# B10532021/Part-Aware_Measurement_for_3D_Pose_Estimation_and_Tracking

Hardware: AMD Instinct MI355X
Metric: multi-view frames/sec (end-to-end: HRNet-W48 2D pose + part-aware cross-view matching + DLT tracking) (higher is better)
Workload: dtype bf16 convs / f64 matching

## Files before the change

include/pam.h:

```cpp
#ifndef PAM_H
#define PAM_H

#include <stddef.h>
#include <stdint.h>

#ifdef __cplusplus
extern "C" {
#endif

#define PAM_J 17
#define PAM_MAX_VIEWS 32
#define PAM_MAX_TAPS 16
#define PAM_EXP_TABLE 64
#define PAM_YOLO_MAX_CAND 1024

#define PAM_OK 0
#define PAM_E_ARG (-1)
#define PAM_E_HIP (-2)
#define PAM_E_STATE (-3)
#define PAM_E_OVERFLOW (-4)

typedef struct PamParams {
    double conf_threshold;
    double epi_threshold;
// ... 105 lines not shown
                            const int32_t* dev_view_of, const float* dev_boxes, int out_h, int out_w, int out_c, void* dev_out_bf16,
                            int antialias);
int pam_preprocess_crops_flip(void* stream, int n, int n_total, const void* const* dev_frames, int frame_h, int frame_w,
                              const int32_t* dev_view_of, const float* dev_boxes, int out_h, int out_w, int out_c, void* dev_out_bf16,
                              int antialias);
int pam_preprocess_crops_affine(void* stream, int n, int n_total, int flip, const void* const* dev_frames, int frame_h, int frame_w,
                                const int32_t* dev_view_of, const float* dev_boxes, float box_scale, int out_h, int out_w, int out_c,
                                void* dev_out_bf16, int antialias, float* dev_eff_xywh);
int pam_box_cs(void* stream, int n, const float* dev_boxes, int out_w, int out_h, float box_scale, float* dev_eff_xywh);
int pam_box_cs_host(int n, const float* boxes, int out_w, int out_h, float box_scale, float* eff);
#define PAM_FLIP_MERGE 1
#define PAM_FLIP_SHIFT 2
#define PAM_FLIP_QUARTER 4
long long pam_head_decode_flip_scratch_bytes(int n, int hm_h, int hm_w);
int pam_head_decode_flip(void* stream, int n, int flip_row0, int hm_h, int hm_w, const void* feat_bf16, int C, const float* w,
                         const float* bias, int J, int flags, float* dev_heatmaps_or_null, const int32_t* dev_view_of,
                         const int32_t* dev_slot_of, const float* dev_boxes, int max_dets, double* dev_det, float* dev_kp_xyc,
                         void* dev_scratch);
long long pam_head_decode_dark_scratch_bytes(int n, int hm_h, int hm_w);
int pam_head_decode_dark(void* stream, int n, int flip_row0, int hm_h, int hm_w, const void* feat_bf16, int C, const float* w,
                         const float* bias, int J, int flags, int blur_kernel, float* dev_heatmaps_or_null, const int32_t* dev_view_of,
                         const int32_t* dev_slot_of, const float* dev_boxes, int max_dets, double* dev_det, float* dev_kp_xyc,
                         void* dev_scratch);
int pam_decode_heatmaps(void* stream, int n, const float* dev_heatmaps, int nchw, int hm_h, int hm_w,
                        const int32_t* dev_view_of, const int32_t* dev_slot_of, const float* dev_boxes,
                        int max_dets, double* dev_det, float* dev_kp_xyc );
int pam_clock_probe(void* stream, unsigned long long* dev_out2, int microseconds);

int pam_conv2d_nhwc_bf16(void* stream, const void* in, const void* w_packed, const void* w_img, const float* bias,
                         const void* residual, void* out, int N, int H, int W, int Cin, int Cout, int KH, int KW,
                         int stride, int pad, int relu, int tile_cfg);
int pam_conv2d_nhwc_bf16_ex(void* stream, const void* in, const void* w_packed, const void* w_img, const float* bias,
                            const void* residual, void* out, int N, int H, int W, int Cin, int Cout, int KH, int KW,
                            int stride, int pad, int relu, int tile_cfg, int in_cstride, int relu_from);
int pam_conv3x3_slab(int H, int W, int Cin, int Cout);
int pam_conv3x3_layout(int H, int W, int Cin, int Cout);
int pam_conv3x3_layout_ex(int H, int W, int Cin, int Cout, int c96_slab);
int pam_conv3x3_layout_gen(int H, int W, int Cin, int Cout);
int pam_conv3x3_layout_small(int H, int W, int Cin, int Cout);
#define PAM_CONV_KERNEL_IGEMM 0
#define PAM_CONV_KERNEL_3X3   1
#define PAM_CONV_KERNEL_3X3S  2
#define PAM_CONV_KERNEL_GS    3
#define PAM_CONV_KERNEL_STEM  4
int pam_conv_last_kernel(void);
int pam_conv_last_form(void);
int pam_conv_plan(int N, int H, int W, int Cin, int Cout, int KH, int KW, int stride, int pad, int relu, int tile_cfg, int in_cstride,
                  int relu_from, int has_in, int has_w_packed, int has_w_img, int has_residual, int has_out, int32_t* kernel, int32_t* form);
int pam_conv_debug_stamps(void* dev_buf);
int pam_upsample_add_nhwc_bf16(void* stream, const void* base, int n_terms, const void* const* terms,
                               const int32_t* shifts, void* out, int N, int H, int W, int C, int relu);
int pam_upsample_add_nhwc_bf16_ex(void* stream, const void* base, int n_terms, const void* const* terms, const int32_t* shifts,
                                  const int32_t* term_cstrides, void* out, int N, int H, int W, int C, int relu);

int pam_basic_block2_tile(int C, int N, int H, int W, int32_t* out2);
int pam_basic_block2_nhwc_bf16(void* stream, const void* in, const void* wpack, void* out, int N, int H, int W, int C,
                               int tile_rows, int tile_cols);

int pam_stem_fused_nhwc_bf16(void* stream, const void* in, const void* w1frag, const float* bias1, const void* w2img, const float* bias2,
                             const void* wp_img, const float* biasp, void* out_x0, void* out_y1, int N, int H, int W);
int pam_bottleneck_fused_nhwc_bf16(void* stream, const void* y1, const void* x0, const void* residual, const void* w2img,
                                   const float* bias2, const void* w3_img, const float* bias3, const void* w1_img, const float* bias1,
                                   void* out_x, void* out_y1, int N, int H, int W);
int pam_resnet_stem_nhwc_bf16(void* stream, const void* in, const void* wfrag, const float* bias, void* out, int N, int H, int W);
int pam_deconv4x4s2_nhwc_bf16(void* stream, const void* in, const void* wimg, const float* bias, void* out, int N, int H, int W,
                              int Cin, int Cout, int relu);
int pam_pointwise64_relu_nhwc_bf16(void* stream, const void* in, const void* w_img, const float* bias, void* out, long long n_pixels);
int pam_pointwise64_act_nhwc_bf16(void* stream, const void* in, const void* w_img, const float* bias, void* out, long long n_pixels, int act);
int pam_bottleneck_tail_nhwc_bf16(void* stream, const void* y2, const void* x0, const void* residual, const void* w3_img,
                                  const float* bias3, const void* w1_img, const float* bias1, void* out_x, void* out_y1,
                                  long long n_pixels, int tile_cfg);

int pam_conv3x3s2_c48_tile(int N, int H, int W, int Cout, int32_t* out3);
int pam_conv3x3s2_slab(int H, int W, int Cin, int Cout);
int pam_conv3x3s2_nhwc_bf16(void* stream, const void* in, int in_cstride, const void* w_img, const float* bias, void* out, int N, int H,
                            int W, int Cin, int Cout, int relu, int relu_from);
int pam_conv3x3s2_c48_nhwc_bf16(void* stream, const void* in, int in_cstride, const void* wpack, const float* bias, const void* res,
                                int res_cstride, void* out, int out_cstride, int N, int H, int W, int Cout, int relu, int relu_from,
                                int tile_rows, int tile_cols, int slab_groups);
int pam_fuse_sum_nhwc_bf16(void* stream, const void* base, int n_plain, const void* const* plain, const int32_t* plain_cstrides, int n_up,
                           const void* const* up_src, const int32_t* up_shifts, const int32_t* up_channels, const void* const* up_wimg,
                           const float* const* up_bias, void* out, int N, int H, int W, int C, int relu, int tile_a, int tile_b,
                           int max_workgroups);

int pam_flag_signal(void* stream, int32_t* dev_counter);
int pam_flag_signal_mask(void* stream, int32_t* dev_counters, uint32_t mask);
int pam_flag_gate(void* stream, int32_t* dev_counter, int target, int32_t* dev_err, const uint32_t* dev_max_us, int arrive, int32_t* host_err,
                  int32_t* dev_void);

int pam_comm_unique_id(void* id128);
int pam_comm_init(void** comm, int world, int rank, const void* id128, int device);
int pam_comm_destroy(void* comm);
const char* pam_comm_last_error(void);
int pam_allgather_keypoints(PamHandle* h, void* comm, void* stream, const double* dev_send, int rows_per_rank, double* dev_recv);

int pam_resize_frames(void* stream, int n, const void* const* dev_frames, int frame_h, int frame_w,
                      int out_h, int out_w, void* dev_out_bf16);
int pam_upsample_concat_nhwc_bf16(void* stream, const void* a, const void* b, void* out, int N, int H, int W, int Ca, int Cb);
int pam_yolo_detect(void* stream, int n_img, const void* const* heads , const int32_t* grid_h,
                    const int32_t* grid_w, const int32_t* chan_stride, const float* anchors, int net_w, int net_h,
                    int num_classes, int class_id, float score_thresh, float nms_thresh, int frame_w, int frame_h,
                    int max_det, float* dev_out, int32_t* dev_count);
long long pam_yolo_detect_workspace_bytes(int n_img, const int32_t* grid_h, const int32_t* grid_w);
int pam_yolo_detect_ws(void* stream, int n_img, const void* const* heads, const int32_t* grid_h, const int32_t* grid_w,
                       const int32_t* chan_stride, const float* anchors, int net_w, int net_h, int num_classes, int class_id,
                       float score_thresh, float nms_thresh, int frame_w, int frame_h, int max_det, float* dev_out, int32_t* dev_count,
                       void* dev_workspace, long long workspace_bytes);

long long pam_yolo_detect_heads_workspace_bytes(int n_img, int n_heads, const int32_t* grid_h, const int32_t* grid_w);
int pam_yolo_detect_heads(void* stream, int n_img, int n_heads, const void* const* heads, const int32_t* grid_h, const int32_t* grid_w,
                          const int32_t* chan_stride, const float* anchors, int net_w, int net_h, int num_classes, int class_id,
                          float score_thresh, float nms_thresh, int frame_w, int frame_h, int max_det, float* dev_out, int32_t* dev_count);
int pam_yolo_detect_heads_ws(void* stream, int n_img, int n_heads, const void* const* heads, const int32_t* grid_h, const int32_t* grid_w,
                             const int32_t* chan_stride, const float* anchors, int net_w, int net_h, int num_classes, int class_id,
                             float score_thresh, float nms_thresh, int frame_w, int frame_h, int max_det, float* dev_out, int32_t* dev_count,
                             void* dev_workspace, long long workspace_bytes);
int pam_maxpool_nhwc_bf16(void* stream, const void* in, void* out, int N, int H, int W, int C, int size, int stride);
#define PAM_SPP_MAX_HW 32
int pam_spp_concat_nhwc_bf16(void* stream, const void* in, void* out, int N, int H, int W, int C, int s1, int s2, int s3);
int pam_spp_concat_slab_nhwc_bf16(void* stream, const void* in, void* out, int N, int H, int W, int C, int s1, int s2, int s3, int slab);

#define PAM_JPEG_U_NOT_JPEG 1
#define PAM_JPEG_U_PROGRESSIVE 2
#define PAM_JPEG_U_ARITHMETIC 3
#define PAM_JPEG_U_SOF 4
#define PAM_JPEG_U_PRECISION 5
#define PAM_JPEG_U_QUANT16 6
#define PAM_JPEG_U_COMPONENTS 7
#define PAM_JPEG_U_COLORSPACE 8
#define PAM_JPEG_U_SAMPLING 9
#define PAM_JPEG_U_SCAN 10
#define PAM_JPEG_U_DNL 11

typedef struct PamJpegInfo {
    int32_t width, height, n_comp;
    int32_t unsupported;
    int32_t h_samp[3], v_samp[3];
    int32_t mcu_w, mcu_h;
    int32_t blocks_w[3], blocks_h[3];
    int32_t restart_interval;
    int32_t reserved;
    int64_t coef_offset[3];
    int64_t coef_words;
    uint16_t quant[3][64];
} PamJpegInfo;

int pam_jpeg_probe(const uint8_t* data, size_t n, PamJpegInfo* info);
int pam_jpeg_entropy(const uint8_t* data, size_t n, const PamJpegInfo* info, int16_t* coef, size_t coef_words);

typedef struct PamJpegImage {
    const int16_t* dev_coef;
    const uint16_t* dev_quant;
    uint8_t* dev_planes;
    uint8_t* dev_out;
    int32_t width, height, n_comp, h_samp, v_samp, reserved;
} PamJpegImage;

int pam_jpeg_reconstruct(void* stream, int n_img, const PamJpegImage* images);


typedef struct PamJpegFwdImage {
    const uint8_t* dev_bgr;
    const uint16_t* dev_quant;
    int16_t* dev_coef;
    int32_t width, height, h_samp, v_samp;
} PamJpegFwdImage;
// ... 46 lines not shown
```

part-aware_measurement_for_3d_pose_estimation_and_tracking_amd/_lib.py:

```python
import ctypes as C
import math
import os

import numpy as np

_HERE = os.path.dirname(os.path.abspath(__file__))
LIB_PATH = os.environ.get('PAM_LIB') or os.path.join(_HERE, 'csrc', 'libpam_hip.so')

PAM_J = 17
PAM_MAX_TAPS = 16
PAM_EXP_TABLE = 64


class PamParams(C.Structure):
    _fields_ = [
        ('conf_threshold', C.c_double), ('epi_threshold', C.c_double), ('init_threshold', C.c_double),
        ('joint_threshold', C.c_double), ('alpha2d', C.c_double), ('lambda_a', C.c_double), ('lambda_t', C.c_double),
        ('n_init', C.c_int32), ('max_age', C.c_int32), ('count_gate', C.c_int32), ('n_taps_body', C.c_int32),
        ('n_taps_arm', C.c_int32), ('reserved', C.c_int32),
        ('taps_body', C.c_double * PAM_MAX_TAPS), ('taps_arm', C.c_double * PAM_MAX_TAPS),
        ('exp_lambda_a', C.c_double * PAM_EXP_TABLE), ('w_lambda_t', C.c_double * 4),
    ]


# ... 26 lines not shown


class PamJpegEncodeParams(C.Structure):
    _fields_ = [('width', C.c_int32), ('height', C.c_int32), ('h_samp', C.c_int32), ('v_samp', C.c_int32),
                ('quality', C.c_int32), ('reserved', C.c_int32), ('quant', (C.c_uint16 * 64) * 2)]


class PamOverlayPrim(C.Structure):
    _fields_ = [('ax', C.c_int32), ('ay', C.c_int32), ('bx', C.c_int32), ('by', C.c_int32), ('hw', C.c_int32), ('bgr', C.c_uint32),
                ('reserved', C.c_int32 * 2)]


class PamOverlayView(C.Structure):
    _fields_ = [('dev_bgr', C.c_void_p), ('width', C.c_int32), ('height', C.c_int32), ('prim_first', C.c_int32), ('prim_count', C.c_int32)]


class PamOverlayTrackView(C.Structure):
    _fields_ = [('camera', C.c_int32), ('extra', C.c_int32), ('width', C.c_int32), ('height', C.c_int32)]


_P = C.c_void_p
_I = C.c_int
_SIGS = {
    'pam_create': (_I, [C.POINTER(_P), _I, _I, _I, _I, _I, _I, C.POINTER(PamParams)]),
    'pam_destroy': (_I, [_P]),
    'pam_last_error': (C.c_char_p, [_P]),
    'pam_version': (C.c_char_p, []),
    'pam_set_cameras': (_I, [_P, _P, _P, _P, _P]),
    'pam_reset': (_I, [_P]),
    'pam_out_layout': (_I, [_P, C.POINTER(PamOutLayout)]),
    'pam_frame_plan': (_I, [_P, _P, _P, _P]),
    'pam_frame': (_I, [_P, _I, _P, _P, _P, _P]),
    'pam_frame_dev': (_I, [_P, _P, _I, _P, _P]),
    'pam_frame_dev_views': (_I, [_P, _P, _I, _P, _P]),
    'pam_fetch': (_I, [_P, _P, _P, _P]),
    'pam_sync': (_I, [_P, _P]),
    'pam_op_project': (_I, [_P, _I, _I, _P, _P]),
    'pam_op_track_affinity': (_I, [_P, _I, _I, _I, _P, _P, _P, _P]),
    'pam_op_lsap': (_I, [_P, _I, _I, _P, _P, _P, _P]),
    'pam_op_epi_dist': (_I, [_P, _I, _P, _P, _P]),
    'pam_op_epi_pair': (_I, [_P, _I, _P, _I, _P, _P]),
    'pam_op_epi_dist_init': (_I, [_P, _I, _P, _P, _P]),
    'pam_op_greedy': (_I, [_P, _I, _I, _P, _P, _P, _P, _P]),
    'pam_op_dlt': (_I, [_P, _I, _P, _P, _P, _P, _P, _P]),
    'pam_op_dlt_paths': (_I, [_P, _I, _P, _P, _P, _P, _P, _I, _I, _P, _P]),
    'pam_op_smooth': (_I, [_P, _I, _P, _P, _P]),
    'pam_op_velocity': (_I, [_P, _I, _P, _P]),
    'pam_op_hyp_cost': (_I, [_P, _I, _P, _P, _I, _P, _P, _P]),
    'pam_preprocess_crops': (_I, [_P, _I, _P, _I, _I, _P, _P, _I, _I, _I, _P]),
    'pam_preprocess_crops_ex': (_I, [_P, _I, _I, _P, _I, _I, _P, _P, _I, _I, _I, _P, _I]),
    'pam_preprocess_crops_flip': (_I, [_P, _I, _I, _P, _I, _I, _P, _P, _I, _I, _I, _P, _I]),
    'pam_preprocess_crops_affine': (_I, [_P, _I, _I, _I, _P, _I, _I, _P, _P, C.c_float, _I, _I, _I, _P, _I, _P]),
    'pam_box_cs': (_I, [_P, _I, _P, _I, _I, C.c_float, _P]),
    'pam_box_cs_host': (_I, [_I, _P, _I, _I, C.c_float, _P]),
    'pam_decode_heatmaps': (_I, [_P, _I, _P, _I, _I, _I, _P, _P, _P, _I, _P, _P]),
    'pam_clock_probe': (_I, [_P, _P, _I]),
    'pam_conv2d_nhwc_bf16': (_I, [_P, _P, _P, _P, _P, _P, _P] + [_I] * 11),
    'pam_conv2d_nhwc_bf16_ex': (_I, [_P, _P, _P, _P, _P, _P, _P] + [_I] * 13),
    'pam_conv3x3_slab': (_I, [_I, _I, _I, _I]),
    'pam_conv3x3_layout': (_I, [_I, _I, _I, _I]),
    'pam_conv_last_kernel': (_I, []),
    'pam_conv_last_form': (_I, []),
    'pam_conv_plan': (_I, [_I] * 18 + [_P, _P]),
    'pam_conv3x3_layout_ex': (_I, [_I, _I, _I, _I, _I]),
    'pam_conv3x3_layout_gen': (_I, [_I, _I, _I, _I]),
    'pam_conv3x3_layout_small': (_I, [_I, _I, _I, _I]),
    'pam_conv_debug_stamps': (_I, [_P]),
    'pam_upsample_add_nhwc_bf16': (_I, [_P, _P, _I, _P, _P, _P, _I, _I, _I, _I, _I]),
    'pam_upsample_add_nhwc_bf16_ex': (_I, [_P, _P, _I, _P, _P, _P, _P, _I, _I, _I, _I, _I]),
    'pam_basic_block2_tile': (_I, [_I, _I, _I, _I, _P]),
    'pam_basic_block2_nhwc_bf16': (_I, [_P, _P, _P, _P, _I, _I, _I, _I, _I, _I]),
    'pam_pointwise64_relu_nhwc_bf16': (_I, [_P, _P, _P, _P, _P, C.c_longlong]),
    'pam_pointwise64_act_nhwc_bf16': (_I, [_P, _P, _P, _P, _P, C.c_longlong, _I]),
    'pam_stem_fused_nhwc_bf16': (_I, [_P] * 10 + [_I, _I, _I]),
    'pam_bottleneck_fused_nhwc_bf16': (_I, [_P] * 12 + [_I, _I, _I]),
    'pam_resnet_stem_nhwc_bf16': (_I, [_P] * 5 + [_I, _I, _I]),
    'pam_deconv4x4s2_nhwc_bf16': (_I, [_P] * 5 + [_I] * 6),
    'pam_bottleneck_tail_nhwc_bf16': (_I, [_P, _P, _P, _P, _P, _P, _P, _P, _P, _P, C.c_longlong, _I]),
    'pam_conv3x3s2_c48_tile': (_I, [_I, _I, _I, _I, _P]),
    'pam_conv3x3s2_c48_nhwc_bf16': (_I, [_P, _P, _I, _P, _P, _P, _I, _P, _I] + [_I] * 9),
    'pam_conv3x3s2_slab': (_I, [_I, _I, _I, _I]),
    'pam_conv3x3s2_nhwc_bf16': (_I, [_P, _P, _I, _P, _P, _P] + [_I] * 7),
    'pam_fuse_sum_nhwc_bf16': (_I, [_P, _P, _I, _P, _P, _I, _P, _P, _P, _P, _P, _P] + [_I] * 8),
    'pam_flag_signal': (_I, [_P, _P]),
    'pam_flag_signal_mask': (_I, [_P, _P, C.c_uint32]),
    'pam_flag_gate': (_I, [_P, _P, _I, _P, _P, _I, _P, _P]),
    'pam_set_input_guard': (_I, [_P, _P]),
    'pam_track_boxes': (_I, [_P, _P, _I, _I, _I, _I, C.c_float, C.c_float, C.c_float, _I, _I, _P, _P, _P, _P]),
    'pam_crop_table': (_I, [_P, _I, _P, _P, _P, _I, _I, _I, _I, _I, _P, _P, _P, _P, _P]),
    'pam_pose_nms': (_I, [_P, _I, _I, _I, _P, _P, _I, _P, _P, _P, _P, C.c_longlong, C.c_longlong, _P, _P, C.c_double, C.c_double, _P, _P, _P]),
    'pam_undistort_keypoints': (_I, [_P, _I, _I, _I, _P, _P, _P, _P, _P]),
    'pam_set_lens': (_I, [_P, _P]),
    'pam_set_one_euro': (_I, [_P, C.POINTER(PamOneEuro)]),
    'pam_one_euro': (_I, [_P, _P, _I, _P, _P]),
    'pam_op_one_euro': (_I, [_P, _I, _I, _P, _P, C.POINTER(PamOneEuro), _P]),
    'pam_comm_unique_id': (_I, [_P]),
    'pam_comm_init': (_I, [C.POINTER(_P), _I, _I, _P, _I]),
    'pam_comm_destroy': (_I, [_P]),
    'pam_comm_last_error': (C.c_char_p, []),
    'pam_allgather_keypoints': (_I, [_P, _P, _P, _P, _I, _P]),
    'pam_head_decode_scratch_bytes': (C.c_longlong, [_I, _I, _I]),
    'pam_head_decode': (_I, [_P, _I, _I, _I, _P, _I, _P, _P, _I, _P, _P, _P, _P, _I, _P, _P, _P]),
    'pam_head_decode_soft_scratch_bytes': (C.c_longlong, [_I, _I, _I]),
    'pam_head_decode_soft': (_I, [_P, _I, _I, _I, _P, _I, _P, _P, _I, C.c_float, _P, _P, _P, _P, _I, _P, _P, _P]),
    'pam_head_decode_flip_scratch_bytes': (C.c_longlong, [_I, _I, _I]),
    'pam_head_decode_flip': (_I, [_P, _I, _I, _I, _I, _P, _I, _P, _P, _I, _I, _P, _P, _P, _P, _I, _P, _P, _P]),
    'pam_head_decode_dark_scratch_bytes': (C.c_longlong, [_I, _I, _I]),
    'pam_head_decode_dark': (_I, [_P, _I, _I, _I, _I, _P, _I, _P, _P, _I, _I, _I, _P, _P, _P, _P, _I, _P, _P, _P]),
    'pam_head_heatmaps': (_I, [_P, _I, _P, _I, _P, _P, _I, _P]),
    'pam_resize_frames': (_I, [_P, _I, _P, _I, _I, _I, _I, _P]),
    'pam_upsample_concat_nhwc_bf16': (_I, [_P, _P, _P, _P, _I, _I, _I, _I, _I]),
    'pam_yolo_detect': (_I, [_P, _I, _P, _P, _P, _P, _P, _I, _I, _I, _I, C.c_float, C.c_float, _I, _I, _I, _P, _P]),
    'pam_yolo_detect_ws': (_I, [_P, _I, _P, _P, _P, _P, _P, _I, _I, _I, _I, C.c_float, C.c_float, _I, _I, _I, _P, _P, _P, C.c_longlong]),
    'pam_yolo_detect_workspace_bytes': (C.c_longlong, [_I, _P, _P]),
    'pam_yolo_detect_heads': (_I, [_P, _I, _I, _P, _P, _P, _P, _P, _I, _I, _I, _I, C.c_float, C.c_float, _I, _I, _I, _P, _P]),
    'pam_yolo_detect_heads_ws': (_I, [_P, _I, _I, _P, _P, _P, _P, _P, _I, _I, _I, _I, C.c_float, C.c_float, _I, _I, _I, _P, _P, _P, C.c_longlong]),
    'pam_yolo_detect_heads_workspace_bytes': (C.c_longlong, [_I, _I, _P, _P]),
    'pam_maxpool_nhwc_bf16': (_I, [_P, _P, _P, _I, _I, _I, _I, _I, _I]),
    'pam_spp_concat_nhwc_bf16': (_I, [_P, _P, _P, _I, _I, _I, _I, _I, _I, _I]),
    'pam_spp_concat_slab_nhwc_bf16': (_I, [_P, _P, _P, _I, _I, _I, _I, _I, _I, _I, _I]),
    'pam_jpeg_probe': (_I, [_P, C.c_size_t, C.POINTER(PamJpegInfo)]),
    'pam_jpeg_entropy': (_I, [_P, C.c_size_t, C.POINTER(PamJpegInfo), _P, C.c_size_t]),
    'pam_jpeg_reconstruct': (_I, [_P, _I, C.POINTER(PamJpegImage)]),
    'pam_jpeg_forward': (_I, [_P, _I, C.POINTER(PamJpegFwdImage)]),
    'pam_jpeg_quality_tables': (_I, [_I, _P]),
    'pam_jpeg_encode_bound': (_I, [_I, _I, _I, _I, C.POINTER(C.c_size_t)]),
    'pam_jpeg_encode': (_I, [_P, C.c_size_t, C.POINTER(PamJpegEncodeParams), _P, C.c_size_t, C.POINTER(C.c_size_t)]),
    'pam_overlay_draw': (_I, [_P, _I, C.POINTER(PamOverlayView), _P, _I]),
    'pam_overlay_draw_counted': (_I, [_P, _I, C.POINTER(PamOverlayView), _P, _I, _P]),
    'pam_overlay_tracks': (_I, [_P, _P, _I, _I, C.POINTER(PamOverlayTrackView), _P, _I, _P, _P, _I, _I, _P, _P]),
}
EXPORTS = tuple(_SIGS)
YOLO_MAX_CAND = 1024
SPP_MAX_HW = 32

TRACK_BOX_RULE = dict(grow=1.25, pad_px=8.0, min_size_px=8.0, max_gap=3)
CROP_CUT_VIEW, CROP_CUT_CAP = 1, 2
POSE_NMS_MAX = 32
COCO_SIGMAS = np.array([.26, .25, .25, .35, .35, .79, .79, .72, .72, .62, .62, 1.07, 1.07, .87, .87, .89, .89]) / 10.0
OKS_VARS = (COCO_SIGMAS * 2) ** 2
LENS_WORDS = 10
LENS_ITERS, LENS_TOL = 8, 1e-9
ONE_EURO_3D = dict(freq=25, mincutoff=0.8, beta=0.4, dcutoff=0.4)
JPEG_MAX_IMAGES = 32
OVERLAY_MAX_VIEWS = 32
OVERLAY_TRACK_ROWS = 36
JPEG_UNSUPPORTED = {1: 'not a JPEG', 2: 'progressive', 3: 'arithmetic coding', 4: 'SOF1 / lossless / differential frame',
                    5: 'sample precision other than 8 bits', 6: '16-bit quantisation table', 7: 'neither one nor three components',
                    8: 'three components that are not YCbCr', 9: 'sampling other than 4:4:4, 4:2:2, 4:2:0', 10: 'not one interleaved scan',
                    11: 'zero height / DNL'}


def one_euro_config(cfg):
    if cfg is None or cfg is False:
        return None
    if isinstance(cfg, PamOneEuro):
        cfg = dict(freq=cfg.freq, mincutoff=cfg.mincutoff, beta=cfg.beta, dcutoff=cfg.dcutoff)
    v = dict(ONE_EURO_3D)
    if cfg is not True:
        for k, x in dict(cfg).items():
            if str(k).lower() not in v:
                raise ValueError('one_euro: unknown key %r (freq, mincutoff, beta, dcutoff)' % (k,))
            v[str(k).lower()] = x
    v = {k: float(x) for k, x in v.items()}
    if not all(math.isfinite(x) for x in v.values()) or v['freq'] <= 0 or v['mincutoff'] <= 0 or v['dcutoff'] <= 0:
        raise ValueError('one_euro: values must be finite, freq, mincutoff and dcutoff > 0 (got %r)' % (v,))
# ... 469 lines not shown
```

part-aware_measurement_for_3d_pose_estimation_and_tracking_amd/csrc/pam_fuse.hip:

```cpp
#include <hip/hip_runtime.h>
#include <stdint.h>
#include "../../include/pam.h"
#include "pam_kernel.hpp"

namespace {

constexpr int FS_MAXI = 5;

struct FSArgs {
    const uint16_t* base; uint16_t* out;
    const uint16_t* plain[2]; int plain_cs[2]; int nplain;
    const uint16_t* src[3]; const char* wimg[3]; const float* ubias[3]; int shift[3]; int src_c[3]; int nup;
    int N, H, W, relu, TA, TB, tiles_y, tiles_x, ntiles, OTH, OTW, smax;
    int w_off[3], w_bytes[3];
    int bias_off;
    int src_off[3], src_bytes;
    int src_base, term_off[3];
    float inv_otw;
};

template <int C>
__global__ __launch_bounds__(576) void k_fuse_sum(FSArgs a) {
    constexpr int C8 = C / 8, NT = C / 16;
    extern __shared__ __attribute__((aligned(1024))) char smem[];
    const int tid = threadIdx.x, lane = tid & 63, g = lane >> 4, l15 = lane & 15;
    const int wave = __builtin_amdgcn_readfirstlane(tid >> 6);
    const int per_img = a.tiles_y * a.tiles_x;

    for (int s = 0; s < a.nup; ++s) {
        {
            const char* wsrc = a.wimg[s] + lane * 16;
            for (int p = wave; p * 1024 < a.w_bytes[s]; p += 9)
                __builtin_amdgcn_global_load_lds((glb_void*)(wsrc + p * 1024), (lds_void*)(smem + a.w_off[s] + p * 1024), 16, 0, 0);
            float* bs = (float*)(smem + a.bias_off) + s * C;
            if (tid < C) bs[tid] = a.ubias[s] ? a.ubias[s][tid] : 0.0f;
        }
    }
    auto src_dma = [&](int T, int b) {
        const int n = T / per_img, trem = T - n * per_img, ty = trem / a.tiles_x, tx = trem - ty * a.tiles_x;
        char* dst0 = smem + a.src_base + b * a.src_bytes;
        for (int s = 0; s < a.nup; ++s) {
            {
                const int sh = a.shift[s], d = a.smax - sh, th = a.TA << d, tw = a.TB << d, Cs = a.src_c[s];
                const int Hs = a.H >> sh, Ws = a.W >> sh, sy0 = (ty * a.TA) << d, sx0 = (tx * a.TB) << d;
                const int rowb = min(tw, Ws - sx0) * Cs * 2, pitch = tw * Cs * 2, npc = (rowb + 1023) >> 10;
                for (int r = 0; r < th && sy0 + r < Hs; ++r)
                    for (int k = 0; k < npc; ++k)
                        if (k * 1024 + lane * 16 < rowb)
                            __builtin_amdgcn_global_load_lds((glb_void*)((const char*)a.src[s] + ((((size_t)n * Hs + sy0 + r) * Ws + sx0) * Cs) * 2 + k * 1024 + lane * 16),
                                                             (lds_void*)(dst0 + a.src_off[s] + r * pitch + k * 1024), 16, 0, 0);
            }
        }
    };
    const int nitem = a.OTH * a.OTW * C8;
    int trc[FS_MAXI];
#pragma unroll
    for (int k = 0; k < FS_MAXI; ++k) {
        const int e = tid + 512 * k;
        const int pix = e / C8, c8 = e - pix * C8;
        const int r = fdiv_small(pix, a.inv_otw), c = pix - r * a.OTW;
        trc[k] = (tid < 512 && e < nitem) ? (r << 16) | (c << 8) | c8 : -1;
    }
    int job0[4];
    {
        int acc_j = 0;
#pragma unroll
        for (int q = 0; q < 3; ++q) {
            job0[q] = acc_j;
            if (q < a.nup) {
                const int d = a.smax - a.shift[a.nup - 1 - q];
                acc_j += ((((a.TA << d) * (a.TB << d)) + 15) >> 4) * NT;
            }
        }
        job0[3] = acc_j;
    }

    int T = (int)blockIdx.x;
    if (wave == 8) {
        if (T < a.ntiles) src_dma(T, 0);
        for (int it = 0; T < a.ntiles; T += (int)gridDim.x, ++it) {
            asm volatile("s_waitcnt vmcnt(0)\n\ts_barrier" ::: "memory");
            if (T + (int)gridDim.x < a.ntiles) src_dma(T + (int)gridDim.x, (it + 1) & 1);
            asm volatile("s_barrier" ::: "memory");
        }
        return;
    }
    asm volatile("s_waitcnt vmcnt(0)" ::: "memory");
    for (int it = 0; T < a.ntiles; T += (int)gridDim.x, ++it) {
        asm volatile("s_waitcnt lgkmcnt(0)\n\ts_barrier" ::: "memory");
        const int n = T / per_img, trem = T - n * per_img, ty = trem / a.tiles_x, tx = trem - ty * a.tiles_x;
        const int oy0 = ty * a.OTH, ox0 = tx * a.OTW;
        bf16x8 vb[FS_MAXI], vp[2][FS_MAXI];
        int eo[FS_MAXI];
#pragma unroll
        for (int k = 0; k < FS_MAXI; ++k) {
            const int r = trc[k] >> 16, c = (trc[k] >> 8) & 255;
            const int oy = oy0 + r, ox = ox0 + c;
            const bool ok = trc[k] >= 0 && oy < a.H && ox < a.W;
            const int p = (n * a.H + oy) * a.W + ox;
            eo[k] = ok ? p : -1;
            const long pz = ok ? p : 0;
            const int c8 = ok ? trc[k] & 255 : 0;
            vb[k] = *(const bf16x8*)(a.base + pz * C + c8 * 8);
#pragma unroll
            for (int t = 0; t < 2; ++t)
                vp[t][k] = t < a.nplain ? *(const bf16x8*)(a.plain[t] + pz * a.plain_cs[t] + c8 * 8) : (bf16x8){0, 0, 0, 0, 0, 0, 0, 0};
        }
        const char* sbuf = smem + a.src_base + (it & 1) * a.src_bytes;
        for (int job = wave; job < job0[3]; job += 8) {
            const int q = job >= job0[2] ? 2 : (job >= job0[1] ? 1 : 0);
            const int s = a.nup - 1 - q, jj = job - job0[q];
            const int mt = jj / NT, j = jj - mt * NT;
            const int d = a.smax - a.shift[s], npx = (a.TA << d) * (a.TB << d);
            const int Cs = a.src_c[s], KS = Cs >> 5;
            const int p = mt * 16 + l15, pq = min(p, npx - 1);
            const char* xp = sbuf + a.src_off[s] + pq * Cs * 2 + g * 16;
            const char* wp = smem + a.w_off[s] + (j * KS * 64 + lane) * 16;
            f32x4 acc = *(const f32x4*)(smem + a.bias_off + (s * C + 16 * j + 4 * g) * 4);
            for (int k0 = 0; k0 < KS; k0 += 3) {
                bf16x8 fa[3], fb[3];
#pragma unroll
                for (int u = 0; u < 3; ++u) {
                    const int ks = min(k0 + u, KS - 1);
                    fa[u] = *(const bf16x8*)(wp + ks * 1024); fb[u] = *(const bf16x8*)(xp + ks * 64);
                }
#pragma unroll
                for (int u = 0; u < 3; ++u)
                    if (k0 + u < KS)
                        acc = __builtin_amdgcn_mfma_f32_16x16x32_bf16(__builtin_bit_cast(bf16x8_t, fa[u]), __builtin_bit_cast(bf16x8_t, fb[u]), acc, 0, 0, 0);
            }
            if (p < npx)
                *(u32x2*)(smem + a.term_off[s] + (p * C + 16 * j + 4 * g) * 2) = (u32x2){pack_bf16x2(acc[0], acc[1]), pack_bf16x2(acc[2], acc[3])};
        }
        asm volatile("s_waitcnt lgkmcnt(0)\n\ts_barrier" ::: "memory");

#pragma unroll
        for (int k = 0; k < FS_MAXI; ++k) {
            if (eo[k] < 0) continue;
            const int r = trc[k] >> 16, c = (trc[k] >> 8) & 255, c8 = trc[k] & 255;
            float v[8];
#pragma unroll
            for (int e = 0; e < 8; ++e) v[e] = bf16_to_f32((uint16_t)vb[k][e]);
#pragma unroll
            for (int t = 0; t < 2; ++t)
                if (t < a.nplain) {
#pragma unroll
                    for (int e = 0; e < 8; ++e) v[e] += bf16_to_f32((uint16_t)vp[t][k][e]);
                }
#pragma unroll
            for (int s = 0; s < 3; ++s)
                if (s < a.nup) {
                    const int sh = a.shift[s], tw = a.TB << (a.smax - sh);
                    const bf16x8 q = *(const bf16x8*)(smem + a.term_off[s] + (((r >> sh) * tw + (c >> sh)) * C + c8 * 8) * 2);
#pragma unroll
                    for (int e = 0; e < 8; ++e) v[e] += bf16_to_f32((uint16_t)q[e]);
                }
            bf16x8 o;
#pragma unroll
            for (int e = 0; e < 8; ++e) o[e] = (short)f32_to_bf16(a.relu ? fmaxf(v[e], 0.0f) : v[e]);
            *(bf16x8*)(a.out + (long)eo[k] * C + c8 * 8) = o;
        }
    }
}

template <int C>
int launch_fs(hipStream_t s, const FSArgs& a, size_t lds, int grid) {
    if (!pam_max_dynamic_lds((const void*)k_fuse_sum<C>, 160 * 1024)) return PAM_E_HIP;
    pam_launch(k_fuse_sum<C>, dim3(grid), dim3(576), lds, s, a);
    return hipGetLastError() == hipSuccess ? PAM_OK : PAM_E_HIP;
}

}

extern "C" int pam_fuse_sum_nhwc_bf16(void* stream, const void* base, int n_plain, const void* const* plain, const int32_t* plain_cstrides,
                                      int n_up, const void* const* up_src, const int32_t* up_shifts, const int32_t* up_channels,
                                      const void* const* up_wimg, const float* const* up_bias, void* out, int N, int H, int W, int C,
                                      int relu, int tile_a, int tile_b, int max_workgroups) {
    if (!base || !out || N < 1 || H < 1 || W < 1 || (C != 48 && C != 96 && C != 192) || n_plain < 0 || n_plain > 2 || n_up < 1 || n_up > 3) return PAM_E_ARG;
    if ((size_t)N * H * W >= (1ull << 31)) return PAM_E_ARG;
    FSArgs a;
    a.base = (const uint16_t*)base; a.out = (uint16_t*)out; a.nplain = n_plain; a.nup = n_up;
    for (int t = 0; t < 2; ++t) {
        a.plain[t] = t < n_plain ? (const uint16_t*)plain[t] : nullptr;
        a.plain_cs[t] = (t < n_plain && plain_cstrides && plain_cstrides[t] > 0) ? plain_cstrides[t] : C;
        if (t < n_plain && (!a.plain[t] || a.plain_cs[t] < C || a.plain_cs[t] % 8 != 0)) return PAM_E_ARG;
    }
    int prev = 0;
    for (int s = 0; s < 3; ++s) {
        const bool on = s < n_up;
        a.src[s] = on ? (const uint16_t*)up_src[s] : nullptr; a.wimg[s] = on ? (const char*)up_wimg[s] : nullptr;
        a.ubias[s] = (on && up_bias) ? up_bias[s] : nullptr; a.shift[s] = on ? up_shifts[s] : 0; a.src_c[s] = on ? up_channels[s] : 0;
        a.w_off[s] = a.w_bytes[s] = a.src_off[s] = a.term_off[s] = 0;
        if (!on) continue;
        if (!a.src[s] || !a.wimg[s] || a.shift[s] <= prev || a.shift[s] > 5 || a.src_c[s] < 32 || a.src_c[s] % 32 != 0) return PAM_E_ARG;
        if (H % (1 << a.shift[s]) != 0 || W % (1 << a.shift[s]) != 0) return PAM_E_ARG;
        prev = a.shift[s];
    }
    a.smax = a.shift[n_up - 1];
    a.N = N; a.H = H; a.W = W; a.relu = relu ? 1 : 0;
    const int c8 = C / 8;
    size_t lds = 0;
    auto plan = [&](int TA, int TB) {
        if ((long)(TA << a.smax) * (TB << a.smax) * c8 > 512L * FS_MAXI || (TA << a.smax) > 32767 || (TB << a.smax) > 255) return false;
        size_t o = 0;
        for (int s = 0; s < n_up; ++s) { a.w_off[s] = (int)o; a.w_bytes[s] = C * a.src_c[s] * 2; o += (size_t)a.w_bytes[s]; }
        a.bias_off = (int)o; o += (size_t)n_up * C * 4; o = (o + 1023) / 1024 * 1024;
        size_t sb = 0;
        for (int s = 0; s < n_up; ++s) { const int d = a.smax - a.shift[s]; a.src_off[s] = (int)sb; sb += (size_t)(TA << d) * (TB << d) * a.src_c[s] * 2; sb = (sb + 1023) / 1024 * 1024; }
        a.src_bytes = (int)sb; a.src_base = (int)o; o += 2 * sb;
        for (int s = 0; s < n_up; ++s) { const int d = a.smax - a.shift[s]; a.term_off[s] = (int)o; o += (size_t)(TA << d) * (TB << d) * C * 2; o = (o + 15) / 16 * 16; }
        lds = o;
        return o <= 160 * 1024;
    };
    int TA = tile_a, TB = tile_b;
    if (TA <= 0 || TB <= 0) {
        const int Hc = H >> a.smax, Wc = W >> a.smax;
        const int cand[8][2] = {{8, 12}, {4, 6}, {4, 3}, {2, 3}, {1, 3}, {1, 2}, {1, 1}, {0, 0}};
        TA = 0;
        for (int pass = 0; pass < 2 && TA == 0; ++pass)
            for (int k = 0; cand[k][0] && TA == 0; ++k)
                if ((pass == 1 || (Hc % cand[k][0] == 0 && Wc % cand[k][1] == 0)) && plan(cand[k][0], cand[k][1])) { TA = cand[k][0]; TB = cand[k][1]; }
        if (TA == 0) return PAM_E_ARG;
    }
    if (!plan(TA, TB)) return PAM_E_ARG;
    a.TA = TA; a.TB = TB; a.OTH = TA << a.smax; a.OTW = TB << a.smax;
    a.tiles_y = (H + a.OTH - 1) / a.OTH; a.tiles_x = (W + a.OTW - 1) / a.OTW;
    const long long nt = (long long)N * a.tiles_y * a.tiles_x;
    if (nt >= (1ll << 30)) return PAM_E_ARG;
    a.ntiles = (int)nt;
    a.inv_otw = 1.0f / (float)a.OTW;
    int ncu = 256;
    {
        static thread_local int cached_dev = -1, cached_cu = 256;
        int dev = 0;
        if (hipGetDevice(&dev) == hipSuccess) {
            if (dev != cached_dev) {
                hipDeviceProp_t pr;
                if (hipGetDeviceProperties(&pr, dev) == hipSuccess && pr.multiProcessorCount > 0) { cached_cu = pr.multiProcessorCount; cached_dev = dev; }
            }
            ncu = cached_cu;
        }
    }
    int grid = max_workgroups > 0 && max_workgroups < ncu ? max_workgroups : ncu;
    const int per_wg = (a.ntiles + grid - 1) / grid;
    grid = (a.ntiles + per_wg - 1) / per_wg;
    switch (C) {
        case 48: return launch_fs<48>((hipStream_t)stream, a, lds, grid);
        case 96: return launch_fs<96>((hipStream_t)stream, a, lds, grid);
        default: return launch_fs<192>((hipStream_t)stream, a, lds, grid);
    }
}
```

Before: 467.6.

## Specialize fuse-sum kernel on plain-input count and search tile plan by cost

```diff
diff --git a/include/pam.h b/include/pam.h
--- a/include/pam.h
+++ b/include/pam.h
@@ -211,6 +211,9 @@
                            const void* const* up_src, const int32_t* up_shifts, const int32_t* up_channels, const void* const* up_wimg,
                            const float* const* up_bias, void* out, int N, int H, int W, int C, int relu, int tile_a, int tile_b,
                            int max_workgroups);
+#define PAM_FUSE_PREFETCH_NONE 0
+#define PAM_FUSE_PREFETCH_REGISTERS 1
+int pam_fuse_sum_last_plan(int32_t* out8);
 
 int pam_flag_signal(void* stream, int32_t* dev_counter);
 int pam_flag_signal_mask(void* stream, int32_t* dev_counters, uint32_t mask);
diff --git a/part-aware_measurement_for_3d_pose_estimation_and_tracking_amd/_lib.py b/part-aware_measurement_for_3d_pose_estimation_and_tracking_amd/_lib.py
--- a/part-aware_measurement_for_3d_pose_estimation_and_tracking_amd/_lib.py
+++ b/part-aware_measurement_for_3d_pose_estimation_and_tracking_amd/_lib.py
@@ -132,6 +132,7 @@
     'pam_conv3x3s2_slab': (_I, [_I, _I, _I, _I]),
     'pam_conv3x3s2_nhwc_bf16': (_I, [_P, _P, _I, _P, _P, _P] + [_I] * 7),
     'pam_fuse_sum_nhwc_bf16': (_I, [_P, _P, _I, _P, _P, _I, _P, _P, _P, _P, _P, _P] + [_I] * 8),
+    'pam_fuse_sum_last_plan': (_I, [_P]),
     'pam_flag_signal': (_I, [_P, _P]),
     'pam_flag_signal_mask': (_I, [_P, _P, C.c_uint32]),
     'pam_flag_gate': (_I, [_P, _P, _I, _P, _P, _I, _P, _P]),
diff --git a/part-aware_measurement_for_3d_pose_estimation_and_tracking_amd/csrc/pam_fuse.hip b/part-aware_measurement_for_3d_pose_estimation_and_tracking_amd/csrc/pam_fuse.hip
--- a/part-aware_measurement_for_3d_pose_estimation_and_tracking_amd/csrc/pam_fuse.hip
+++ b/part-aware_measurement_for_3d_pose_estimation_and_tracking_amd/csrc/pam_fuse.hip
@@ -5,7 +5,11 @@
 
 namespace {
 
-constexpr int FS_MAXI = 5;
+#ifdef PAM_FS_PREFETCH
+constexpr int fs_maxi(int n_plain) { return n_plain == 0 ? 5 : 3; }
+#else
+constexpr int fs_maxi(int n_plain) { return n_plain == 0 ? 7 : 5; }
+#endif
 
 struct FSArgs {
     const uint16_t* base; uint16_t* out;
@@ -19,22 +23,25 @@
     float inv_otw;
 };
 
-template <int C>
+template <int NP>
+struct FSTile { bf16x8 b[fs_maxi(NP)]; bf16x8 p[NP > 0 ? NP : 1][fs_maxi(NP)]; };
+
+template <int C, int NP>
 __global__ __launch_bounds__(576) void k_fuse_sum(FSArgs a) {
-    constexpr int C8 = C / 8, NT = C / 16;
+    constexpr int C8 = C / 8, NT = C / 16, FS_MAXI = fs_maxi(NP);
     extern __shared__ __attribute__((aligned(1024))) char smem[];
     const int tid = threadIdx.x, lane = tid & 63, g = lane >> 4, l15 = lane & 15;
     const int wave = __builtin_amdgcn_readfirstlane(tid >> 6);
-    const int per_img = a.tiles_y * a.tiles_x;
+    const int per_img = a.tiles_y * a.tiles_x, G = (int)gridDim.x;
 
     for (int s = 0; s < a.nup; ++s) {
-        {
-            const char* wsrc = a.wimg[s] + lane * 16;
-            for (int p = wave; p * 1024 < a.w_bytes[s]; p += 9)
-                __builtin_amdgcn_global_load_lds((glb_void*)(wsrc + p * 1024), (lds_void*)(smem + a.w_off[s] + p * 1024), 16, 0, 0);
-            float* bs = (float*)(smem + a.bias_off) + s * C;
-            if (tid < C) bs[tid] = a.ubias[s] ? a.ubias[s][tid] : 0.0f;
-        }
+#ifndef PAM_KO_FS_FILL
+        const char* wsrc = a.wimg[s] + lane * 16;
+        for (int p = wave; p * 1024 < a.w_bytes[s]; p += 9)
+            __builtin_amdgcn_global_load_lds((glb_void*)(wsrc + p * 1024), (lds_void*)(smem + a.w_off[s] + p * 1024), 16, 0, 0);
+#endif
+        float* bs = (float*)(smem + a.bias_off) + s * C;
+        if (tid < C) bs[tid] = a.ubias[s] ? a.ubias[s][tid] : 0.0f;
     }
     auto src_dma = [&](int T, int b) {
         const int n = T / per_img, trem = T - n * per_img, ty = trem / a.tiles_x, tx = trem - ty * a.tiles_x;
@@ -76,36 +83,81 @@
     }
 
     int T = (int)blockIdx.x;
+    if (T >= a.ntiles) return;
     if (wave == 8) {
-        if (T < a.ntiles) src_dma(T, 0);
-        for (int it = 0; T < a.ntiles; T += (int)gridDim.x, ++it) {
+        src_dma(T, 0);
+        for (int it = 0; T < a.ntiles; T += G, ++it) {
             asm volatile("s_waitcnt vmcnt(0)\n\ts_barrier" ::: "memory");
-            if (T + (int)gridDim.x < a.ntiles) src_dma(T + (int)gridDim.x, (it + 1) & 1);
+            if (T + G < a.ntiles) src_dma(T + G, (it + 1) & 1);
             asm volatile("s_barrier" ::: "memory");
         }
         return;
     }
-    asm volatile("s_waitcnt vmcnt(0)" ::: "memory");
-    for (int it = 0; T < a.ntiles; T += (int)gridDim.x, ++it) {
-        asm volatile("s_waitcnt lgkmcnt(0)\n\ts_barrier" ::: "memory");
-        const int n = T / per_img, trem = T - n * per_img, ty = trem / a.tiles_x, tx = trem - ty * a.tiles_x;
-        const int oy0 = ty * a.OTH, ox0 = tx * a.OTW;
-        bf16x8 vb[FS_MAXI], vp[2][FS_MAXI];
-        int eo[FS_MAXI];
+    const int img_px = a.H * a.W;
+    auto item_pixel = [&](int k, int oy0, int ox0) __attribute__((always_inline)) {
+        const int oy = oy0 + (trc[k] >> 16), ox = ox0 + ((trc[k] >> 8) & 255);
+        return (trc[k] >= 0 && oy < a.H && ox < a.W) ? oy * a.W + ox : -1;
+    };
+    auto fetch = [&](int Tq, bool on, FSTile<NP>& R) __attribute__((always_inline)) {
+        const int n = Tq / per_img, trem = Tq - n * per_img, ty = trem / a.tiles_x, tx = trem - ty * a.tiles_x;
+#ifndef PAM_KO_FS_BASE
+        const auto rs_b = __builtin_amdgcn_make_buffer_rsrc((void*)(a.base + (size_t)n * img_px * C), 0, img_px * C * 2, 0x00020000);
+        __amdgpu_buffer_rsrc_t rs_p[NP > 0 ? NP : 1];
+#pragma unroll
+        for (int t = 0; t < NP; ++t)
+            rs_p[t] = __builtin_amdgcn_make_buffer_rsrc((void*)(a.plain[t] + (size_t)n * img_px * a.plain_cs[t]), 0, ((img_px - 1) * a.plain_cs[t] + C) * 2, 0x00020000);
+#endif
 #pragma unroll
         for (int k = 0; k < FS_MAXI; ++k) {
-            const int r = trc[k] >> 16, c = (trc[k] >> 8) & 255;
-            const int oy = oy0 + r, ox = ox0 + c;
-            const bool ok = trc[k] >= 0 && oy < a.H && ox < a.W;
-            const int p = (n * a.H + oy) * a.W + ox;
-            eo[k] = ok ? p : -1;
-            const long pz = ok ? p : 0;
-            const int c8 = ok ? trc[k] & 255 : 0;
-            vb[k] = *(const bf16x8*)(a.base + pz * C + c8 * 8);
-#pragma unroll
-            for (int t = 0; t < 2; ++t)
-                vp[t][k] = t < a.nplain ? *(const bf16x8*)(a.plain[t] + pz * a.plain_cs[t] + c8 * 8) : (bf16x8){0, 0, 0, 0, 0, 0, 0, 0};
-        }
+            const int p = item_pixel(k, ty * a.OTH, tx * a.OTW);
+            const bool ok = on && p >= 0;
+            const int c8 = trc[k] & 255;
+#ifdef PAM_KO_FS_BASE
+            R.b[k] = (bf16x8){(short)(ok ? p : 0), (short)c8, 0, 0, 0, 0, 0, 0};
+#pragma unroll
+            for (int t = 0; t < NP; ++t) R.p[t][k] = R.b[k];
+#else
+            R.b[k] = __builtin_bit_cast(bf16x8, __builtin_amdgcn_raw_buffer_load_b128(rs_b, ok ? (unsigned)(p * C + c8 * 8) * 2u : OOB_OFFSET, 0, 0));
+#pragma unroll
+            for (int t = 0; t < NP; ++t)
+                R.p[t][k] = __builtin_bit_cast(bf16x8, __builtin_amdgcn_raw_buffer_load_b128(rs_p[t], ok ? (unsigned)(p * a.plain_cs[t] + c8 * 8) * 2u : OOB_OFFSET, 0, 0));
+#endif
+        }
+    };
+    auto sum_store = [&](int Tq, const FSTile<NP>& R) __attribute__((always_inline)) {
+#ifndef PAM_KO_FS_SUM
+        const int n = Tq / per_img, trem = Tq - n * per_img, ty = trem / a.tiles_x, tx = trem - ty * a.tiles_x;
+        const auto rs_o = __builtin_amdgcn_make_buffer_rsrc((void*)(a.out + (size_t)n * img_px * C), 0, img_px * C * 2, 0x00020000);
+#pragma unroll
+        for (int k = 0; k < FS_MAXI; ++k) {
+            const int p = item_pixel(k, ty * a.OTH, tx * a.OTW);
+            const int tk = trc[k] >= 0 ? trc[k] : 0;
+            const int r = tk >> 16, c = (tk >> 8) & 255, c8 = tk & 255;
+            float v[8];
+#pragma unroll
+            for (int e = 0; e < 8; ++e) v[e] = bf16_to_f32((uint16_t)R.b[k][e]);
+#pragma unroll
+            for (int t = 0; t < NP; ++t) {
+#pragma unroll
+                for (int e = 0; e < 8; ++e) v[e] += bf16_to_f32((uint16_t)R.p[t][k][e]);
+            }
+#pragma unroll
+            for (int s = 0; s < 3; ++s)
+                if (s < a.nup) {
+                    const int sh = a.shift[s], tw = a.TB << (a.smax - sh);
+                    const bf16x8 q = *(const bf16x8*)(smem + a.term_off[s] + (((r >> sh) * tw + (c >> sh)) * C + c8 * 8) * 2);
+#pragma unroll
+                    for (int e = 0; e < 8; ++e) v[e] += bf16_to_f32((uint16_t)q[e]);
+                }
+            bf16x8 o;
+#pragma unroll
+            for (int e = 0; e < 8; ++e) o[e] = (short)f32_to_bf16(a.relu ? fmaxf(v[e], 0.0f) : v[e]);
+            __builtin_amdgcn_raw_buffer_store_b128(__builtin_bit_cast(u32x4, o), rs_o, p >= 0 ? (unsigned)(p * C + c8 * 8) * 2u : OOB_OFFSET, 0, 0);
+        }
+#endif
+    };
+    auto products = [&](int it) __attribute__((always_inline)) {
+#ifndef PAM_KO_FS_PROD
         const char* sbuf = smem + a.src_base + (it & 1) * a.src_bytes;
         for (int job = wave; job < job0[3]; job += 8) {
             const int q = job >= job0[2] ? 2 : (job >= job0[1] ? 1 : 0);
@@ -132,42 +184,50 @@
             if (p < npx)
                 *(u32x2*)(smem + a.term_off[s] + (p * C + 16 * j + 4 * g) * 2) = (u32x2){pack_bf16x2(acc[0], acc[1]), pack_bf16x2(acc[2], acc[3])};
         }
+#endif
+    };
+    auto step = [&](int Tq, int it, FSTile<NP>& cur, FSTile<NP>& nxt) __attribute__((always_inline)) {
         asm volatile("s_waitcnt lgkmcnt(0)\n\ts_barrier" ::: "memory");
-
-#pragma unroll
-        for (int k = 0; k < FS_MAXI; ++k) {
-            if (eo[k] < 0) continue;
-            const int r = trc[k] >> 16, c = (trc[k] >> 8) & 255, c8 = trc[k] & 255;
-            float v[8];
-#pragma unroll
-            for (int e = 0; e < 8; ++e) v[e] = bf16_to_f32((uint16_t)vb[k][e]);
-#pragma unroll
-            for (int t = 0; t < 2; ++t)
-                if (t < a.nplain) {
-#pragma unroll
-                    for (int e = 0; e < 8; ++e) v[e] += bf16_to_f32((uint16_t)vp[t][k][e]);
-                }
-#pragma unroll
-            for (int s = 0; s < 3; ++s)
-                if (s < a.nup) {
-                    const int sh = a.shift[s], tw = a.TB << (a.smax - sh);
-                    const bf16x8 q = *(const bf16x8*)(smem + a.term_off[s] + (((r >> sh) * tw + (c >> sh)) * C + c8 * 8) * 2);
-#pragma unroll
-                    for (int e = 0; e < 8; ++e) v[e] += bf16_to_f32((uint16_t)q[e]);
-                }
-            bf16x8 o;
-#pragma unroll
-            for (int e = 0; e < 8; ++e) o[e] = (short)f32_to_bf16(a.relu ? fmaxf(v[e], 0.0f) : v[e]);
-            *(bf16x8*)(a.out + (long)eo[k] * C + c8 * 8) = o;
-        }
-    }
-}
-
+#ifdef PAM_FS_PREFETCH
+        const bool more = Tq + G < a.ntiles;
+        fetch(more ? Tq + G : Tq, more, nxt);
+#else
+        fetch(Tq, true, cur);
+#endif
+        products(it);
+        asm volatile("s_waitcnt lgkmcnt(0)\n\ts_barrier" ::: "memory");
+        sum_store(Tq, cur);
+    };
+    FSTile<NP> r0, r1;
+#ifdef PAM_FS_PREFETCH
+    fetch(T, true, r0);
+#endif
+    __builtin_amdgcn_s_waitcnt(0x0F70);
+    for (int it = 0;; it += 2) {
+        step(T, it, r0, r1);
+        T += G;
+        if (T >= a.ntiles) break;
+        step(T, it + 1, r1, r0);
+        T += G;
+        if (T >= a.ntiles) break;
+    }
+}
+
+thread_local int32_t fs_last_plan[8] = {0, 0, 0, 0, 0, 0, 0, 0};
+
+template <int C, int NP>
+int launch_fs(hipStream_t s, const FSArgs& a, size_t lds, int grid) {
+    if (!pam_max_dynamic_lds((const void*)k_fuse_sum<C, NP>, 160 * 1024)) return PAM_E_HIP;
+    pam_launch(k_fuse_sum<C, NP>, dim3(grid), dim3(576), lds, s, a);
+    return hipGetLastError() == hipSuccess ? PAM_OK : PAM_E_HIP;
+}
 template <int C>
-int launch_fs(hipStream_t s, const FSArgs& a, size_t lds, int grid) {
-    if (!pam_max_dynamic_lds((const void*)k_fuse_sum<C>, 160 * 1024)) return PAM_E_HIP;
-    pam_launch(k_fuse_sum<C>, dim3(grid), dim3(576), lds, s, a);
-    return hipGetLastError() == hipSuccess ? PAM_OK : PAM_E_HIP;
+int launch_fs_c(hipStream_t s, const FSArgs& a, size_t lds, int grid) {
+    switch (a.nplain) {
+        case 0: return launch_fs<C, 0>(s, a, lds, grid);
+        case 1: return launch_fs<C, 1>(s, a, lds, grid);
+        default: return launch_fs<C, 2>(s, a, lds, grid);
+    }
 }
 
 }
@@ -184,6 +244,7 @@
         a.plain[t] = t < n_plain ? (const uint16_t*)plain[t] : nullptr;
         a.plain_cs[t] = (t < n_plain && plain_cstrides && plain_cstrides[t] > 0) ? plain_cstrides[t] : C;
         if (t < n_plain && (!a.plain[t] || a.plain_cs[t] < C || a.plain_cs[t] % 8 != 0)) return PAM_E_ARG;
+        if ((size_t)H * W * a.plain_cs[t] * 2 >= (1ull << 31)) return PAM_E_ARG;
     }
     int prev = 0;
     for (int s = 0; s < 3; ++s) {
@@ -198,37 +259,6 @@
     }
     a.smax = a.shift[n_up - 1];
     a.N = N; a.H = H; a.W = W; a.relu = relu ? 1 : 0;
-    const int c8 = C / 8;
-    size_t lds = 0;
-    auto plan = [&](int TA, int TB) {
-        if ((long)(TA << a.smax) * (TB << a.smax) * c8 > 512L * FS_MAXI || (TA << a.smax) > 32767 || (TB << a.smax) > 255) return false;
-        size_t o = 0;
-        for (int s = 0; s < n_up; ++s) { a.w_off[s] = (int)o; a.w_bytes[s] = C * a.src_c[s] * 2; o += (size_t)a.w_bytes[s]; }
-        a.bias_off = (int)o; o += (size_t)n_up * C * 4; o = (o + 1023) / 1024 * 1024;
-        size_t sb = 0;
-        for (int s = 0; s < n_up; ++s) { const int d = a.smax - a.shift[s]; a.src_off[s] = (int)sb; sb += (size_t)(TA << d) * (TB << d) * a.src_c[s] * 2; sb = (sb + 1023) / 1024 * 1024; }
-        a.src_bytes = (int)sb; a.src_base = (int)o; o += 2 * sb;
-        for (int s = 0; s < n_up; ++s) { const int d = a.smax - a.shift[s]; a.term_off[s] = (int)o; o += (size_t)(TA << d) * (TB << d) * C * 2; o = (o + 15) / 16 * 16; }
-        lds = o;
-        return o <= 160 * 1024;
-    };
-    int TA = tile_a, TB = tile_b;
-    if (TA <= 0 || TB <= 0) {
-        const int Hc = H >> a.smax, Wc = W >> a.smax;
-        const int cand[8][2] = {{8, 12}, {4, 6}, {4, 3}, {2, 3}, {1, 3}, {1, 2}, {1, 1}, {0, 0}};
-        TA = 0;
-        for (int pass = 0; pass < 2 && TA == 0; ++pass)
-            for (int k = 0; cand[k][0] && TA == 0; ++k)
-                if ((pass == 1 || (Hc % cand[k][0] == 0 && Wc % cand[k][1] == 0)) && plan(cand[k][0], cand[k][1])) { TA = cand[k][0]; TB = cand[k][1]; }
-        if (TA == 0) return PAM_E_ARG;
-    }
-    if (!plan(TA, TB)) return PAM_E_ARG;
-    a.TA = TA; a.TB = TB; a.OTH = TA << a.smax; a.OTW = TB << a.smax;
-    a.tiles_y = (H + a.OTH - 1) / a.OTH; a.tiles_x = (W + a.OTW - 1) / a.OTW;
-    const long long nt = (long long)N * a.tiles_y * a.tiles_x;
-    if (nt >= (1ll << 30)) return PAM_E_ARG;
-    a.ntiles = (int)nt;
-    a.inv_otw = 1.0f / (float)a.OTW;
     int ncu = 256;
     {
         static thread_local int cached_dev = -1, cached_cu = 256;
@@ -241,12 +271,64 @@
             ncu = cached_cu;
         }
     }
-    int grid = max_workgroups > 0 && max_workgroups < ncu ? max_workgroups : ncu;
-    const int per_wg = (a.ntiles + grid - 1) / grid;
-    grid = (a.ntiles + per_wg - 1) / per_wg;
+    const int cap = max_workgroups > 0 && max_workgroups < ncu ? max_workgroups : ncu;
+    auto walk = [&](int TA, int TB) {
+        const long long nt = (long long)N * ((H + (TA << a.smax) - 1) / (TA << a.smax)) * ((W + (TB << a.smax) - 1) / (TB << a.smax));
+        return nt >= (1ll << 30) ? 0 : (int)((nt + cap - 1) / cap);
+    };
+    const int c8 = C / 8;
+    const long max_px = 512L * fs_maxi(n_plain) / c8;
+    size_t lds = 0;
+    auto plan = [&](int TA, int TB) {
+        if ((long)(TA << a.smax) * (TB << a.smax) > max_px || (TA << a.smax) > 32767 || (TB << a.smax) > 255 || walk(TA, TB) < 1) return false;
+        size_t o = 0;
+        for (int s = 0; s < n_up; ++s) { a.w_off[s] = (int)o; a.w_bytes[s] = C * a.src_c[s] * 2; o += (size_t)a.w_bytes[s]; }
+        a.bias_off = (int)o; o += (size_t)n_up * C * 4; o = (o + 1023) / 1024 * 1024;
+        size_t sb = 0;
+        for (int s = 0; s < n_up; ++s) { const int d = a.smax - a.shift[s]; a.src_off[s] = (int)sb; sb += (size_t)(TA << d) * (TB << d) * a.src_c[s] * 2; sb = (sb + 1023) / 1024 * 1024; }
+        a.src_bytes = (int)sb; a.src_base = (int)o; o += (walk(TA, TB) > 1 ? 2 : 1) * sb;
+        for (int s = 0; s < n_up; ++s) { const int d = a.smax - a.shift[s]; a.term_off[s] = (int)o; o += (size_t)(TA << d) * (TB << d) * C * 2; o = (o + 15) / 16 * 16; }
+        lds = o;
+        return o <= 160 * 1024;
+    };
+    int TA = tile_a, TB = tile_b;
+    if (TA <= 0 || TB <= 0) {
+        const int Hc = H >> a.smax, Wc = W >> a.smax, unit = 1 << (2 * a.smax);
+        const long lim = max_px / unit;
+        long long best = -1;
+        TA = 0;
+        for (int ta = 1; ta <= Hc && ta <= lim; ++ta)
+            for (int tb = (int)(lim / ta < Wc ? lim / ta : Wc); tb >= 1; --tb) {
+                const int wk = walk(ta, tb);
+                if (wk < 1) continue;
+                const long long ntl = (long long)N * ((Hc + ta - 1) / ta) * ((Wc + tb - 1) / tb);
+                const long long cost = ((long long)wk << 44) + ntl * ((long long)ta * tb * unit + 9600 / C);
+                if ((best < 0 || cost < best) && plan(ta, tb)) { best = cost; TA = ta; TB = tb; }
+            }
+        if (TA == 0) return PAM_E_ARG;
+    }
+    if (!plan(TA, TB)) return PAM_E_ARG;
+    a.TA = TA; a.TB = TB; a.OTH = TA << a.smax; a.OTW = TB << a.smax;
+    a.tiles_y = (H + a.OTH - 1) / a.OTH; a.tiles_x = (W + a.OTW - 1) / a.OTW;
+    a.ntiles = N * a.tiles_y * a.tiles_x;
+    a.inv_otw = 1.0f / (float)a.OTW;
+    const int per_wg = walk(TA, TB);
+    const int grid = (a.ntiles + per_wg - 1) / per_wg;
+#ifdef PAM_FS_PREFETCH
+    const int32_t rec[8] = {TA, TB, a.ntiles, grid, per_wg, (int32_t)lds, PAM_FUSE_PREFETCH_REGISTERS, 1};
+#else
+    const int32_t rec[8] = {TA, TB, a.ntiles, grid, per_wg, (int32_t)lds, PAM_FUSE_PREFETCH_NONE, 0};
+#endif
+    for (int k = 0; k < 8; ++k) fs_last_plan[k] = rec[k];
     switch (C) {
-        case 48: return launch_fs<48>((hipStream_t)stream, a, lds, grid);
-        case 96: return launch_fs<96>((hipStream_t)stream, a, lds, grid);
-        default: return launch_fs<192>((hipStream_t)stream, a, lds, grid);
-    }
-}
+        case 48: return launch_fs_c<48>((hipStream_t)stream, a, lds, grid);
+        case 96: return launch_fs_c<96>((hipStream_t)stream, a, lds, grid);
+        default: return launch_fs_c<192>((hipStream_t)stream, a, lds, grid);
+    }
+}
+
+extern "C" int pam_fuse_sum_last_plan(int32_t* out8) {
+    if (!out8) return PAM_E_ARG;
+    for (int k = 0; k < 8; ++k) out8[k] = fs_last_plan[k];
+    return PAM_OK;
+}
```

New measurement: 460.3. 0.984x the previous value.
